# Kloudy-Sky/openintel

Hardware: AMD Instinct MI355X
Metric: queries/sec + p50 latency, 10M-post/768-d hybrid BM25+cosine+RRF top-100 (higher is better)
Workload: dtype f32

## Files before the change

### openintel_amd/csrc/cosine_screen_i8.hip

```cpp
#include <algorithm>
#include <cmath>
#include <cstdlib>
#include <type_traits>

#include "oi_device.h"
#include "oi_internal.h"
#include "oi_screen_stage.h"
#include "oi_lds_dma.h"

typedef int i8s_i32x4 __attribute__((ext_vector_type(4)));
typedef int i8s_i32x16 __attribute__((ext_vector_type(16)));
typedef float i8s_f32x2 __attribute__((ext_vector_type(2)));
template <int N>
struct i8s_ivec {
    typedef int type __attribute__((ext_vector_type(N)));
};

#define I8S_TILE_ROWS 32
#define I8S_SLOT_BYTES (I8S_TILE_ROWS * 128)
#define I8S_META_BYTES 256
#define I8S_PAD_ROWS 64

size_t oi_screen_i8_meta_offset(uint64_t n, uint32_t dim) { return ((size_t)n * dim + 255) & ~(size_t)255; }
size_t oi_screen_i8_bytes(uint64_t n, uint32_t dim) {
    return oi_screen_i8_meta_offset(n, dim) + 8 * ((size_t)n + I8S_PAD_ROWS) + 256;
}

__global__ __launch_bounds__(256) void i8s_make_kernel(const float *__restrict__ rows, uint64_t n, uint32_t dim,
                                                       const uint32_t *__restrict__ long_bitmap, uint32_t *__restrict__ out_i8,
                                                       float *__restrict__ meta, uint32_t *__restrict__ emax_bits) {
    const uint32_t lane = threadIdx.x & 63;
    const uint64_t wave = ((uint64_t)blockIdx.x * blockDim.x + threadIdx.x) >> 6;
    const uint64_t n_waves = ((uint64_t)gridDim.x * blockDim.x) >> 6;
    const uint32_t nv = dim >> 2;
    float best = 0.f;
    for (uint64_t r = wave; r < n; r += n_waves) {
        const float4 *x = reinterpret_cast<const float4 *>(rows + r * dim);
        float4 v[3];
        float amax = 0.f;
#pragma unroll
        for (int u = 0; u < 3; ++u) {
            const uint32_t j = lane + 64u * u;
            v[u] = j < nv ? x[j] : make_float4(0.f, 0.f, 0.f, 0.f);
            amax = fmaxf(amax, fmaxf(fmaxf(fabsf(v[u].x), fabsf(v[u].y)), fmaxf(fabsf(v[u].z), fabsf(v[u].w))));
        }
#pragma unroll
        for (int o = 32; o > 0; o >>= 1) amax = fmaxf(amax, __shfl_xor(amax, o, OI_WAVE));
        const float s = amax / 127.f;
        double e2 = 0.0;
#pragma unroll
        for (int u = 0; u < 3; ++u) {
            const uint32_t j = lane + 64u * u;
            const float xs[4] = {v[u].x, v[u].y, v[u].z, v[u].w};
            uint32_t packed = 0;
#pragma unroll
            for (int c = 0; c < 4; ++c) {
                float t = s > 0.f ? rintf(xs[c] / s) : 0.f;
                t = fminf(127.f, fmaxf(-127.f, t));
                const int iv = (int)t;
                const double e = (double)s * (double)iv - (double)xs[c];
                e2 += j < nv ? e * e : 0.0;
                packed |= ((uint32_t)iv & 0xFFu) << (8 * c);
            }
            if (j < nv) out_i8[r * nv + j] = packed;
        }
        e2 = oi_wave_sum(e2);
        const float er = (float)sqrt(e2) * 1.00000095367431640625f;
        if (lane == 0) {
            meta[2 * r] = s;
            meta[2 * r + 1] = er;
        }
        const bool is_long = long_bitmap && ((long_bitmap[r >> 5] >> (r & 31)) & 1u);
        if (!is_long) best = fmaxf(best, er);
    }
    if (lane == 0) atomicMax(emax_bits, __float_as_uint(best));
}

int oi_launch_make_screen_i8(oi_ctx *ctx, const float *rows, uint64_t n, uint32_t dim, const uint32_t *long_bitmap, uint8_t *out) {
    OI_REQUIRE(oi_cosine_screen_supported(dim), "int8 screening copy: dim %u not instantiated (384, 768)", dim);
    const size_t mo = oi_screen_i8_meta_offset(n, dim);
    OI_HIP_CHECK(hipMemsetAsync(out + mo, 0, 8 * ((size_t)n + I8S_PAD_ROWS) + 256, ctx->stream));
    if (n == 0) return OI_OK;
    uint64_t blocks = (n + 3) / 4;
    const uint64_t cap = (uint64_t)ctx->num_cus * 8;
    if (blocks > cap) blocks = cap;
    float *meta = reinterpret_cast<float *>(out + mo);
    hipLaunchKernelGGL(i8s_make_kernel, dim3((uint32_t)blocks), dim3(256), 0, ctx->stream, rows, n, dim, long_bitmap,
                       reinterpret_cast<uint32_t *>(out), meta, reinterpret_cast<uint32_t *>(meta + 2 * (n + I8S_PAD_ROWS)));
    OI_HIP_CHECK(hipGetLastError());
    return OI_OK;
}

#define I8S_NORM_LIMIT 1.0e15f
#define I8S_QNORM_MIN 1.0e-12f
__device__ __forceinline__ void i8s_stage_query_row(const float *__restrict__ q, uint32_t row, uint32_t n_queries, uint32_t n_padded, uint32_t dim,
                                                    const uint32_t *__restrict__ max_norm_bits, const uint32_t *__restrict__ emax_bits,
                                                    int8_t *__restrict__ qi8, float *__restrict__ qf, uint32_t *gate) {
    const uint32_t lane = threadIdx.x & 63;
    const bool real = row < n_queries;
    float amax = 0.f;
    bool fin = true;
    for (uint32_t k = lane; k < dim; k += 64) {
        const float f = real ? q[(uint64_t)row * dim + k] : 0.f;
        fin = fin && (f - f == 0.f);
        amax = fmaxf(amax, fabsf(f));
    }
#pragma unroll
    for (int o = 32; o > 0; o >>= 1) amax = fmaxf(amax, __shfl_xor(amax, o, OI_WAVE));
    fin = __builtin_amdgcn_ballot_w64(!fin) == 0ull;
    const float a = fin ? amax / 127.f : 0.f;
    double qn2 = 0.0, en2 = 0.0;
    for (uint32_t k = lane; k < dim; k += 64) {
        const float f = real ? q[(uint64_t)row * dim + k] : 0.f;
        float h = 0.f, l = 0.f;
        if (a > 0.f) {
            const float t = f / a;
            h = fminf(127.f, fmaxf(-127.f, rintf(t)));
            l = fminf(127.f, fmaxf(-127.f, rintf((t - h) * 128.f)));
        }
        const double qh = (double)a * ((double)h + (double)l * 0.0078125);
        qn2 += qh * qh;
        en2 += (qh - (double)f) * (qh - (double)f);
        qi8[(uint64_t)row * dim + k] = (int8_t)(int)h;
        qi8[((uint64_t)n_padded + row) * dim + k] = (int8_t)(int)l;
    }
    qn2 = oi_wave_sum(qn2);
    en2 = oi_wave_sum(en2);
    if (lane == 0) {
        const float up = 1.00000095367431640625f;
        const float qn = (float)sqrt(qn2) * up, en = (float)sqrt(en2) * up;
        const float X = __uint_as_float(max_norm_bits[0]), em = __uint_as_float(*emax_bits);
        const bool ok = fin && amax > 0.f && qn < I8S_NORM_LIMIT && qn >= I8S_QNORM_MIN && X < I8S_NORM_LIMIT && em < I8S_NORM_LIMIT;
        const float rnd = 3.814697265625e-06f + (float)dim * 2.384185791015625e-07f;
        const float cq = 1.001f * (X * en + rnd * (X + em) * (qn + en)) + 1.0e-27f;
        const float m2 = 2.002f * (em * qn + cq);
        qf[row] = ok ? a : 0.f;
        qf[n_padded + row] = ok ? qn : 0.f;
        qf[2 * n_padded + row] = ok ? cq : 0.f;
        qf[3 * n_padded + row] = ok || !real ? m2 : __builtin_inff();
        if (real && !ok) *gate = 1u;
    }
}
__global__ __launch_bounds__(256) void i8s_stage_kernel(const float *__restrict__ q, uint32_t n_queries, uint32_t n_padded, uint32_t dim,
                                                        const uint32_t *__restrict__ max_norm_bits, const uint32_t *__restrict__ emax_bits,
                                                        int8_t *__restrict__ qi8, float *__restrict__ qf, uint32_t *gate) {
    const uint32_t wave = (blockIdx.x * blockDim.x + threadIdx.x) >> 6, n_waves = (gridDim.x * blockDim.x) >> 6;
    for (uint32_t row = wave; row < n_padded; row += n_waves) {
        i8s_stage_query_row(q, row, n_queries, n_padded, dim, max_norm_bits, emax_bits, qi8, qf, gate);
    }
}

__global__ __launch_bounds__(256) void i8s_stage_both_kernel(const float *__restrict__ q, uint32_t n_queries, uint32_t n_padded, uint32_t dim,
                                                             const uint32_t *__restrict__ max_norm_bits, const uint32_t *__restrict__ emax_bits,
                                                             int8_t *__restrict__ qi8, float *__restrict__ qf, uint16_t *__restrict__ q_bf16,
                                                             float *__restrict__ eps2, uint32_t *gate) {
    const uint32_t wave = (blockIdx.x * blockDim.x + threadIdx.x) >> 6, n_waves = (gridDim.x * blockDim.x) >> 6;
    for (uint32_t row = wave; row < n_padded; row += n_waves) {
        i8s_stage_query_row(q, row, n_queries, n_padded, dim, max_norm_bits, emax_bits, qi8, qf, gate);
        pf_stage_query_row(q, row, n_queries, dim, max_norm_bits, q_bf16, eps2, gate);
    }
}

int oi_launch_screen_stage_i8(oi_ctx *ctx, const float *d_queries, uint32_t n_queries, uint32_t dim, const uint32_t *max_norm_bits,
                              const uint8_t *i8_copy, uint64_t n_rows, int8_t *qi8, float *qf, uint32_t *gate, uint16_t *q_bf16,
                              float *eps2) {
    const uint32_t n_padded = (n_queries + 31u) & ~31u;
    if (n_padded == 0) return OI_OK;
    const uint32_t *emax = reinterpret_cast<const uint32_t *>(i8_copy + oi_screen_i8_meta_offset(n_rows, dim)) + 2 * (n_rows + I8S_PAD_ROWS);
    if (q_bf16)
        hipLaunchKernelGGL(i8s_stage_both_kernel, dim3((n_padded + 3) / 4), dim3(256), 0, ctx->stream, d_queries, n_queries, n_padded, dim,
                           max_norm_bits, emax, qi8, qf, q_bf16, eps2, gate);
    else
        hipLaunchKernelGGL(i8s_stage_kernel, dim3((n_padded + 3) / 4), dim3(256), 0, ctx->stream, d_queries, n_queries, n_padded, dim,
                           max_norm_bits, emax, qi8, qf, gate);
    OI_HIP_CHECK(hipGetLastError());
    return OI_OK;
}

__device__ __forceinline__ void i8s_issue_piece(const oi_u32x4 &srd, uint32_t voff, uint32_t soff, uint32_t lds_dst) {
#ifdef I8S_NO_DMA
    (void)srd; (void)voff; (void)soff; (void)lds_dst;
#else
    oi_dma_piece(srd, voff, soff, lds_dst);
#endif
}
__device__ __forceinline__ void i8s_issue_meta(const oi_u32x4 &srd, uint32_t voff, uint32_t lds_dst) {
#ifdef I8S_NO_DMA
    (void)srd; (void)voff; (void)lds_dst;
#else
    uint32_t keep;
    const uint32_t d = __builtin_amdgcn_readfirstlane(lds_dst);
    asm volatile(
        "s_mov_b32 %0, m0\n\t"
        "s_mov_b32 m0, %3\n\t"
        "s_nop 0\n\t"
        "buffer_load_dword %1, %2, 0 offen " OI_DMA_NT "lds\n\t"
        "s_mov_b32 m0, %0"
        : "=&s"(keep)
        : "v"(voff), "s"(srd), "s"(d)
        : "memory");
#endif
}

template <int D, int NQT, int NBUF, bool FILT>
__global__ __launch_bounds__(256, 1) void cosine_i8_screen(
    const uint8_t *__restrict__ rows, const float *__restrict__ meta, uint64_t row_begin, uint64_t row_end,
    const int8_t *__restrict__ qhi, const int8_t *__restrict__ qlo,
    const float *__restrict__ qf, uint32_t qf_stride, uint32_t n_queries, uint32_t doc_id_base, uint64_t *pools, uint32_t *seg_cnt,
    uint32_t seg_cnt_stride, const uint32_t *tau_keys, uint64_t pool_stride, uint32_t carry_cap, uint32_t seg_cap, uint32_t *overflow,
    const uint4 *__restrict__ filt, const uint2 *__restrict__ attrs) {
    constexpr int NKC = D / 128;
    constexpr int P = NBUF - 1;
    constexpr int KSTEPS = D / 32;
    constexpr uint32_t RING = NBUF * I8S_SLOT_BYTES;
    static_assert(D % 128 == 0 && P >= 2 && P <= 2 * NKC, "unsupported ring depth for this D");
    constexpr uint32_t QLO_LDS = NQT * KSTEPS * 64 * 16;
    static_assert(NQT * KSTEPS * 4 <= 200, "the hi query block must fit the register file");
    static_assert(4 * RING + 4 * 2 * I8S_META_BYTES + 256 + OI_STAGE_LDS + QLO_LDS <= 160 * 1024, "LDS");

    extern __shared__ __attribute__((aligned(1024))) unsigned char smem[];
    unsigned char *ring = smem;
    unsigned char *meta_lds = smem + 4 * RING;
    uint32_t *seg_fill = reinterpret_cast<uint32_t *>(smem + 4 * RING + 8 * I8S_META_BYTES);
    unsigned char *stage_base = smem + 4 * RING + 8 * I8S_META_BYTES + 256;
    unsigned char *qlo_lds = stage_base + OI_STAGE_LDS;

    OI_CLAIM_WHOLE_SIMD();
    const uint32_t tid = threadIdx.x, lane = tid & 63;
    const uint32_t w = __builtin_amdgcn_readfirstlane(tid >> 6);
    const uint32_t li = lane & 31, lh = lane >> 5;
    uint64_t *stage_keys = reinterpret_cast<uint64_t *>(stage_base) + w * OI_STAGE;
    uint32_t *stage_q = reinterpret_cast<uint32_t *>(stage_base + 4 * OI_STAGE * 8) + w * OI_STAGE;
    uint32_t st_head = 0, st_n = 0;

    i8s_i32x4 qh[NQT][KSTEPS];
#pragma unroll
    for (int t = 0; t < NQT; ++t)
#pragma unroll
        for (int s = 0; s < KSTEPS; ++s)
            qh[t][s] = *reinterpret_cast<const i8s_i32x4 *>(qhi + (uint64_t)(32 * t + li) * D + 32 * s + 16 * lh);
    for (uint32_t c = tid; c < (uint32_t)(NQT * KSTEPS * 64); c += 256) {
        const uint32_t t = c / (KSTEPS * 64), s = (c / 64) % KSTEPS, l = c % 64;
        *reinterpret_cast<i8s_i32x4 *>(qlo_lds + c * 16) =
            *reinterpret_cast<const i8s_i32x4 *>(qlo + (uint64_t)(32 * t + (l & 31)) * D + 32 * s + 16 * (l >> 5));
    }
    float qa[NQT], qn[NQT], cq[NQT], tc[NQT];
#pragma unroll
    for (int t = 0; t < NQT; ++t) {
        const uint32_t q = 32u * t + li;
        const bool real = q < n_queries;
        const uint32_t k = real ? tau_keys[q] : 0xFFFFFFFFu;
        const float tau = k <= 0x007FFFFFu ? -__builtin_inff() : oi_key_f32(k);
        qa[t] = real ? qf[q] * 0.0078125f : 0.f;
        qn[t] = real ? qf[qf_stride + q] : 0.f;
        cq[t] = real ? qf[2 * qf_stride + q] : 0.f;
        const float m2 = real ? qf[3 * qf_stride + q] : 0.f;
        const float T = m2 < __builtin_inff() ? (tau + m2) - (fabsf(tau) + m2) * 9.5367431640625e-07f : -__builtin_inff();
        tc[t] = T - cq[t];
    }
    if (tid < 32 * NQT) seg_fill[tid] = 0;
#ifdef I8S_NO_DMA
    for (uint32_t i = tid; i < (4 * RING + 8 * I8S_META_BYTES) / 4; i += 256) reinterpret_cast<uint32_t *>(smem)[i] = 0u;
#endif
    __syncthreads();

    const uint64_t n_rows = row_end - row_begin;
    const uint64_t n_tiles = (n_rows + I8S_TILE_ROWS - 1) / I8S_TILE_ROWS;
    const uint64_t first = (uint64_t)blockIdx.x * 4 + w, stride = (uint64_t)gridDim.x * 4;
    const uint64_t my_nt = first < n_tiles ? (n_tiles - first + stride - 1) / stride : 0;
    uint64_t *my_seg = pools + carry_cap + (uint64_t)blockIdx.x * seg_cap;

    if (my_nt) {
        uint32_t voff[4];
#pragma unroll
        for (int m = 0; m < 4; ++m) {
            const uint32_t prow = 8 * m + (lane >> 3);
            voff[m] = prow * (uint32_t)D + (((lane & 7) ^ ((prow >> 1) & 7)) << 4);
        }
        const uint32_t ring_w = oi_lds_addr(ring) + w * RING;
        const unsigned char *ring_rd = ring + w * RING;
        const uint32_t meta_w = oi_lds_addr(meta_lds) + w * 2 * I8S_META_BYTES;
        const unsigned char *meta_rd = meta_lds + w * 2 * I8S_META_BYTES;
        uint32_t frag_off[4];
#pragma unroll
        for (int g = 0; g < 4; ++g) frag_off[g] = li * 128 + (((2 * g + lh) ^ ((li >> 1) & 7)) << 4);

        auto tile_row0 = [&](uint64_t ti) { return row_begin + (first + ti * stride) * (uint64_t)I8S_TILE_ROWS; };
        auto tile_srd = [&](uint64_t ti) {
            const uint64_t r0 = tile_row0(ti < my_nt ? ti : 0);
            return oi_make_srd(rows + r0 * D, ti < my_nt ? (row_end - r0) * (uint64_t)D : 0ull);
        };
        auto issue_meta = [&](uint64_t ti) {
            const uint64_t r0 = tile_row0(ti);
            i8s_issue_meta(oi_make_srd(meta + 2 * r0, (row_end - r0) * 8ull), lane * 4u, meta_w + (uint32_t)(ti & 1) * I8S_META_BYTES);
        };
        oi_u32x4 s0 = tile_srd(0), s1 = tile_srd(1), s2 = tile_srd(2);
        __builtin_amdgcn_s_waitcnt(0x0F70);
        oi_static_for<0, P>([&](auto j_) {
            constexpr int j = decltype(j_)::value;
            constexpr int tj = j / NKC, kj = j % NKC;
#pragma unroll
            for (int m = 0; m < 4; ++m)
                i8s_issue_piece(tj == 0 ? s0 : (tj == 1 ? s1 : s2), voff[m], kj * 128, ring_w + j * I8S_SLOT_BYTES + m * 1024);
        });
        issue_meta(0);
        uint32_t rd_off = 0, wr_off = (NBUF - 1) * I8S_SLOT_BYTES;
        auto lo_frag = [&](int t, int s) {
            return *reinterpret_cast<const i8s_i32x4 *>(qlo_lds + ((t * KSTEPS + s) * 64 + lane) * 16);
        };
        i8s_i32x4 b_cur[NQT];
#ifndef I8S_NO_MFMA
#pragma unroll
        for (int t = 0; t < NQT; ++t) b_cur[t] = lo_frag(t, 0);
#endif

        oi_wait_vm<4 * (P - 1)>();
        i8s_i32x4 a_cur = *reinterpret_cast<const i8s_i32x4 *>(ring_rd + frag_off[0]);

        constexpr int NS = 16 * NQT;
        constexpr int RPK = KSTEPS >= 20 ? 1 : 2;
        constexpr int NSL = 16 / RPK, T0 = 4;
        static_assert(T0 + NSL <= KSTEPS, "the tile test does not fit the span");
        static_assert(4 * NKC + 4 >= 4 * (P - 1) - 1, "the ring's wait in k-step 3 must retire the previous tile's metadata");
        typename i8s_ivec<NS>::type S;
#pragma unroll
        for (int i = 0; i < NS; ++i) S[i] = 0;
        i8s_i32x16 ah[NQT], al[NQT];
        i8s_f32x2 md_cur[RPK];
#pragma unroll
        for (int u = 0; u < RPK; ++u) md_cur[u] = i8s_f32x2{0.f, 0.f};
        const uint32_t lh32 = 32u * lh;
        auto meta_row = [&](const unsigned char *mt, int r) {
            return *reinterpret_cast<const i8s_f32x2 *>(mt + lh32 + ((r & 3) + 8 * (r >> 2)) * 8);
        };
        float cap_sc = 0.f, cap_er = 0.f;
        auto test_row = [&](int t, int r, const i8s_f32x2 md) -> uint32_t {
            const float sc = oi_mul_unpacked((float)S[16 * t + r], oi_mul_unpacked(md[0], qa[t]));
            const bool pass = sc >= oi_fma_unpacked(-md[1], qn[t], tc[t]);
            cap_sc = pass ? sc : cap_sc;
            cap_er = pass ? md[1] : cap_er;
            return pass ? 1u << (16 * t + r) : 0u;
        };

        for (uint64_t ti = 0;; ++ti) {
            const bool live = ti < my_nt;
            const unsigned char *mt = meta_rd + (uint32_t)((ti + 1) & 1) * I8S_META_BYTES;
            uint32_t m = 0;
            if (live) {
#pragma unroll
                for (int t = 0; t < NQT; ++t)
#pragma unroll
                    for (int r = 0; r < 16; ++r) { ah[t][r] = 0; al[t][r] = 0; }

                oi_static_for<0, NKC * 4>([&](auto gi_) {
                    constexpr int gi = decltype(gi_)::value;
                    constexpr int kc = gi / 4, g = gi % 4;
                    constexpr int sn = kc + P;
                    constexpr int tn = sn / NKC, kn = sn % NKC;
                    i8s_i32x4 a_nxt;
                    if constexpr (g < 3) {
                        a_nxt = *reinterpret_cast<const i8s_i32x4 *>(ring_rd + rd_off + frag_off[g + 1]);
                    } else {
                        oi_wait_vm<4 * (P - 1) - 1>();
                        const uint32_t nx_off = rd_off + I8S_SLOT_BYTES == RING ? 0u : rd_off + I8S_SLOT_BYTES;
                        a_nxt = *reinterpret_cast<const i8s_i32x4 *>(ring_rd + nx_off + frag_off[0]);
                    }
                    i8s_f32x2 md_nxt[RPK];
                    if constexpr (gi >= T0 - 1 && gi < T0 - 1 + NSL) {
#pragma unroll
                        for (int u = 0; u < RPK; ++u) md_nxt[u] = meta_row(mt, RPK * (gi - (T0 - 1)) + u);
                    }
#ifndef I8S_NO_MFMA
                    i8s_i32x4 b_nxt[NQT];
#pragma unroll
                    for (int t = 0; t < NQT; ++t) b_nxt[t] = lo_frag(t, (gi + 1) % KSTEPS);
#endif
                    __builtin_amdgcn_sched_barrier(0);
#pragma unroll
                    for (int t = 0; t < NQT; ++t) {
#ifndef I8S_NO_MFMA
                        ah[t] = __builtin_amdgcn_mfma_i32_32x32x32_i8(a_cur, qh[t][gi], ah[t], 0, 0, 0);
                        al[t] = __builtin_amdgcn_mfma_i32_32x32x32_i8(a_cur, b_cur[t], al[t], 0, 0, 0);
#else
                        asm volatile("" : : "v"(a_cur));
#endif
                        if constexpr (gi >= T0 && gi < T0 + NSL) if (t == 0) {
#pragma unroll
                            for (int u = 0; u < RPK; ++u)
#pragma unroll
                                for (int tt = 0; tt < NQT; ++tt) m |= test_row(tt, RPK * (gi - T0) + u, md_cur[u]);
                            asm volatile("" : "+v"(m), "+v"(cap_sc), "+v"(cap_er));
                        }
                        __builtin_amdgcn_sched_barrier(0);
                    }
#ifndef I8S_NO_MFMA
#pragma unroll
                    for (int t = 0; t < NQT; ++t) b_cur[t] = b_nxt[t];
#endif
                    if constexpr (gi >= T0 - 1 && gi < T0 - 1 + NSL) {
#pragma unroll
                        for (int u = 0; u < RPK; ++u) md_cur[u] = md_nxt[u];
                    }
                    i8s_issue_piece(tn == 0 ? s0 : (tn == 1 ? s1 : s2), voff[g], kn * 128, ring_w + wr_off + g * 1024);
                    if constexpr (g == 3) {
                        wr_off = rd_off;
                        rd_off = rd_off + I8S_SLOT_BYTES == RING ? 0u : rd_off + I8S_SLOT_BYTES;
                    }
                    a_cur = a_nxt;
                });
            } else {
                oi_wait_vm<0>();
#pragma unroll
                for (int r = 0; r < 16; ++r) {
                    const i8s_f32x2 md = meta_row(mt, r);
#pragma unroll
                    for (int t = 0; t < NQT; ++t) m |= test_row(t, r, md);
                }
            }

            const uint64_t row0 = tile_row0(ti ? ti - 1 : 0);
            if (ti == 0) m = 0u;
            const uint32_t m_tested = m;
            if (row_end - row0 < (uint64_t)I8S_TILE_ROWS) {
                const uint32_t left = (uint32_t)(row_end - row0);
#pragma unroll
                for (int r = 0; r < 16; ++r)
                    if ((uint32_t)((r & 3) + 8 * (r >> 2)) + 4u * lh >= left) m &= ~(0x00010001u << r);
            }
#if defined(I8S_NO_DMA) || defined(I8S_NO_MFMA) || defined(I8S_NO_APPEND)
            if (seg_cap != 0xFFFFFFFFu) m = 0u;
#endif
            if (__builtin_amdgcn_ballot_w64(m != 0u) != 0ull) {
                if constexpr (FILT) m = oi_filter_tile<NQT>(m, filt, attrs, row0, lh, li);
                static_assert(64u <= OI_STAGE - OI_STAGE_FLUSH, "a tile of one pair per lane must fit the staging ring");
                if (__builtin_amdgcn_ballot_w64((m_tested & (m_tested - 1u)) != 0u) == 0ull) {
                    const uint64_t has = __builtin_amdgcn_ballot_w64(m != 0u);
                    if (m != 0u) {
                        const uint32_t bit = (uint32_t)__builtin_ctz(m), r = bit & 15u;
                        const bool t1 = NQT > 1 && bit >= 16u;
                        const uint32_t rit = (r & 3) + 8 * (r >> 2) + 4 * lh;
                        const float low = cap_sc - fmaf(cap_er, t1 ? qn[NQT - 1] : qn[0], t1 ? cq[NQT - 1] : cq[0]);
                        const uint32_t below = __builtin_amdgcn_mbcnt_hi((uint32_t)(has >> 32), __builtin_amdgcn_mbcnt_lo((uint32_t)has, 0u));
                        const uint32_t idx = (st_head + st_n + below) & (OI_STAGE - 1);
                        stage_keys[idx] = oi_rank_key(low, doc_id_base + ((uint32_t)row0 + rit));
                        stage_q[idx] = (t1 ? 32u : 0u) + li;
                    }
                    st_n += (uint32_t)__builtin_popcountll(has);
                    while (st_n >= OI_STAGE_FLUSH) {
                        OI_STAGE_FLUSH_TO_POOL(OI_STAGE_FLUSH);
                    }
                } else {
                    const uint32_t cnt = (uint32_t)__builtin_popcount(m);
                    const uint32_t incl = oi_wave_incl_scan(cnt);
                    const uint32_t total = (uint32_t)__builtin_amdgcn_readlane((int)incl, 63);
                    const uint32_t any = oi_wave_or(m);
                    auto lower_key = [&](int t, uint32_t r) -> uint64_t {
                        const uint32_t rit = (r & 3) + 8 * (r >> 2) + 4 * lh;
                        const i8s_f32x2 md = *reinterpret_cast<const i8s_f32x2 *>(mt + rit * 8);
                        const float sc = (float)S[16 * t + r] * (md[0] * qa[t]);
                        return oi_rank_key(sc - fmaf(md[1], qn[t], cq[t]), doc_id_base + ((uint32_t)row0 + rit));
                    };
                    if (total <= OI_STAGE - OI_STAGE_FLUSH) {
                        uint32_t idx = st_head + st_n + incl - cnt;
#pragma unroll
                        for (int t = 0; t < NQT; ++t)
                            for (uint32_t wd = (any >> (16 * t)) & 0xFFFFu; wd; wd &= wd - 1) {
                                const uint32_t r = (uint32_t)__builtin_ctz(wd);
                                if (m & (1u << (16 * t + r))) {
                                    stage_keys[idx & (OI_STAGE - 1)] = lower_key(t, r);
                                    stage_q[idx & (OI_STAGE - 1)] = 32u * t + li;
                                    ++idx;
                                }
                            }
                        st_n += total;
                        while (st_n >= OI_STAGE_FLUSH) {
                            OI_STAGE_FLUSH_TO_POOL(OI_STAGE_FLUSH);
                        }
                    } else {
                        uint32_t pos[NQT];
#pragma unroll
                        for (int t = 0; t < NQT; ++t)
                            pos[t] = atomicAdd(&seg_fill[32u * t + li], (uint32_t)__builtin_popcount((m >> (16 * t)) & 0xFFFFu));
#pragma unroll
                        for (int t = 0; t < NQT; ++t) {
                            uint64_t *dst = my_seg + (uint64_t)(32u * t + li) * pool_stride;
                            for (uint32_t wd = (any >> (16 * t)) & 0xFFFFu; wd; wd &= wd - 1) {
                                const uint32_t r = (uint32_t)__builtin_ctz(wd);
                                if (m & (1u << (16 * t + r))) {
                                    if (pos[t] < seg_cap) dst[pos[t]] = lower_key(t, r);
                                    else *overflow = 1u;
                                    ++pos[t];
                                }
                            }
                        }
                    }
                }
            }
            if (!live) break;
#pragma unroll
            for (int t = 0; t < NQT; ++t)
#pragma unroll
                for (int r = 0; r < 16; ++r) S[16 * t + r] = ah[t][r] * 128 + al[t][r];
            if (ti + 1 < my_nt) issue_meta(ti + 1);
            s0 = s1;
            s1 = s2;
            s2 = tile_srd(ti + 3);
        }
        if (st_n) {
            OI_STAGE_FLUSH_TO_POOL(st_n);
        }
        oi_wait_vm<0>();
    }
    __syncthreads();
    if (tid < 32 * NQT && tid < n_queries) {
        const uint32_t c = seg_fill[tid];
        seg_cnt[(uint64_t)tid * seg_cnt_stride + blockIdx.x] = c < seg_cap ? c : seg_cap;
    }
}

template <int D, int NQT, int NBUF, bool FILT>
static int launch_i8_screen_k(oi_ctx *ctx, const uint8_t *rows, const float *meta, uint64_t row_begin, uint64_t row_end, const int8_t *qhi,
                              const int8_t *qlo, const float *qf, uint32_t qf_stride, uint32_t nq, uint32_t doc_id_base, const PoolView &p) {
    constexpr size_t smem = 4 * NBUF * I8S_SLOT_BYTES + 8 * I8S_META_BYTES + 256 + OI_STAGE_LDS + NQT * (D / 32) * 64 * 16;
    OI_CHECK(oi_dyn_lds(ctx, reinterpret_cast<const void *>(cosine_i8_screen<D, NQT, NBUF, FILT>), (size_t)(smem)));
    hipLaunchKernelGGL((cosine_i8_screen<D, NQT, NBUF, FILT>), dim3(p.n_segs), dim3(256), smem, ctx->stream, rows, meta, row_begin, row_end,
                       qhi, qlo, qf, qf_stride, nq, doc_id_base, p.keys, p.seg_cnt, p.seg_cnt_stride, p.tau_keys, p.stride, p.carry_cap,
                       p.seg_cap, p.overflow, p.filt, p.attrs);
    OI_HIP_CHECK(hipGetLastError());
    return OI_OK;
}
template <int D, int NQT, int NBUF>
static int launch_i8_screen(oi_ctx *ctx, const uint8_t *rows, const float *meta, uint64_t row_begin, uint64_t row_end, const int8_t *qhi,
                            const int8_t *qlo, const float *qf, uint32_t qf_stride, uint32_t nq, uint32_t doc_id_base, const PoolView &p) {
    return p.filt ? launch_i8_screen_k<D, NQT, NBUF, true>(ctx, rows, meta, row_begin, row_end, qhi, qlo, qf, qf_stride, nq, doc_id_base, p)
                  : launch_i8_screen_k<D, NQT, NBUF, false>(ctx, rows, meta, row_begin, row_end, qhi, qlo, qf, qf_stride, nq, doc_id_base, p);
}

int oi_launch_cosine_screen_i8_chunk(oi_ctx *ctx, const uint8_t *i8_copy, uint64_t n_rows_total, uint64_t row_begin, uint64_t row_end,
                                     uint32_t dim, const int8_t *qi8, const float *qf, uint32_t n_queries, uint32_t doc_id_base,
                                     PoolView &pool) {
    OI_REQUIRE(oi_cosine_screen_supported(dim), "cosine screen (int8): dim %u not instantiated (384, 768)", dim);
    OI_REQUIRE(row_end <= n_rows_total, "cosine screen (int8): rows past the copy");
    oi_cosine_screen_geometry(ctx, row_end > row_begin ? row_end - row_begin : 0, &pool.n_segs, &pool.seg_cap);
    OI_REQUIRE(pool.n_segs <= pool.seg_cnt_stride && pool.carry_cap + (uint64_t)pool.n_segs * pool.seg_cap <= pool.stride,
               "cosine screen (int8): chunk does not fit the candidate pool");
    if (row_end <= row_begin || n_queries == 0) return OI_OK;
    const float *meta = reinterpret_cast<const float *>(i8_copy + oi_screen_i8_meta_offset(n_rows_total, dim));
    const uint32_t np = (n_queries + 31u) & ~31u;
    ProfScope ps(ctx, "cosine");
    for (uint32_t q0 = 0; q0 < n_queries; q0 += 64) {
        const uint32_t nq_here = std::min(64u, n_queries - q0);
        const PoolView p = pool.for_queries(q0);
        const int8_t *qhi = qi8 + (uint64_t)q0 * dim, *qlo = qi8 + ((uint64_t)np + q0) * dim;
        const float *qfp = qf + q0;
        const bool two = nq_here > 32;
        if (dim == 768) {
            if (two) OI_CHECK((launch_i8_screen<768, 2, 6>(ctx, i8_copy, meta, row_begin, row_end, qhi, qlo, qfp, np, nq_here, doc_id_base, p)));
            else OI_CHECK((launch_i8_screen<768, 1, 6>(ctx, i8_copy, meta, row_begin, row_end, qhi, qlo, qfp, np, nq_here, doc_id_base, p)));
        } else {
            if (two) OI_CHECK((launch_i8_screen<384, 2, 6>(ctx, i8_copy, meta, row_begin, row_end, qhi, qlo, qfp, np, nq_here, doc_id_base, p)));
            else OI_CHECK((launch_i8_screen<384, 1, 6>(ctx, i8_copy, meta, row_begin, row_end, qhi, qlo, qfp, np, nq_here, doc_id_base, p)));
        }
    }
    return OI_OK;
}

__device__ __forceinline__ float i8s_bf16_lo(uint32_t w) { return __uint_as_float(w << 16); }
__device__ __forceinline__ float i8s_bf16_hi(uint32_t w) { return __uint_as_float(w & 0xFFFF0000u); }
__global__ __launch_bounds__(256) void pf_rescreen_kernel(const uint16_t *__restrict__ copy, uint64_t n_rows, uint32_t dim,
                                                          uint32_t doc_id_base, const uint16_t *__restrict__ qb, uint64_t *pools,
                                                          const uint32_t *__restrict__ cnt, uint64_t stride, uint32_t cap) {
    const uint32_t q = blockIdx.y, lane = threadIdx.x & 63;
    const uint32_t wave = (blockIdx.x * blockDim.x + threadIdx.x) >> 6, n_waves = (gridDim.x * blockDim.x) >> 6;
    uint32_t c = cnt[q];
    c = c < cap ? c : cap;
    uint64_t *keys = pools + (uint64_t)q * stride;
    const uint32_t nvec = dim >> 3;
    const uint4 *qv = reinterpret_cast<const uint4 *>(qb + (uint64_t)q * dim);
    for (uint32_t i0 = wave * 4u; i0 < c; i0 += n_waves * 4u) {
        uint32_t doc[4];
        const uint4 *x[4];
        float a[4];
#pragma unroll
        for (int u = 0; u < 4; ++u) {
            const uint32_t i = i0 + u < c ? i0 + u : c - 1u;
            doc[u] = oi_rank_key_doc(keys[i]);
            const uint64_t r = (uint64_t)(doc[u] - doc_id_base);
            x[u] = reinterpret_cast<const uint4 *>(copy + (r < n_rows ? r : 0) * dim);
            a[u] = 0.f;
        }
        for (uint32_t v = lane; v < nvec; v += 64) {
            const uint4 yv = qv[v];
            uint4 xv[4];
#pragma unroll
            for (int u = 0; u < 4; ++u) xv[u] = oi_load_stream(x[u] + v);
#pragma unroll
            for (int u = 0; u < 4; ++u) {
                const uint32_t xw[4] = {xv[u].x, xv[u].y, xv[u].z, xv[u].w}, yw[4] = {yv.x, yv.y, yv.z, yv.w};
#pragma unroll
                for (int e = 0; e < 4; ++e) {
                    a[u] = oi_fma_unpacked(i8s_bf16_lo(xw[e]), i8s_bf16_lo(yw[e]), a[u]);
                    a[u] = oi_fma_unpacked(i8s_bf16_hi(xw[e]), i8s_bf16_hi(yw[e]), a[u]);
                }
            }
        }
        float s[4];
#pragma unroll
        for (int u = 0; u < 4; ++u) s[u] = oi_wave_sum(a[u]);
#pragma unroll
        for (int u = 0; u < 4; ++u) {
            const uint64_t r = (uint64_t)(doc[u] - doc_id_base);
            const float sc = r < n_rows ? s[u] : 0.f;
            if (lane == 0 && i0 + u < c) keys[i0 + u] = oi_rank_key(sc, doc[u]);
        }
    }
}

int oi_launch_rescreen_bf16(oi_ctx *ctx, const uint16_t *copy_rows, uint64_t n_rows, uint32_t dim, uint32_t doc_id_base,
                            const uint16_t *q_bf16, uint32_t n_queries, const PoolView &pool) {
    if (n_queries == 0) return OI_OK;
    ProfScope ps(ctx, "rescreen");
    hipLaunchKernelGGL(pf_rescreen_kernel, dim3(32, n_queries), dim3(256), 0, ctx->stream, copy_rows, n_rows, dim, doc_id_base, q_bf16,
                       pool.keys, pool.carry_cnt, pool.stride, pool.carry_cap);
    OI_HIP_CHECK(hipGetLastError());
    return OI_OK;
}
```

### openintel_amd/csrc/select.hip

```cpp
#include "oi_device.h"
#include "oi_internal.h"

#define SEL_THREADS 1024
#define SEL_MAX 1024

__device__ void bitonic_sort_desc(uint64_t *a, uint32_t P) {
    const uint32_t tid = threadIdx.x;
    for (uint32_t size = 2; size <= P; size <<= 1) {
        for (uint32_t stride = size >> 1; stride > 0; stride >>= 1) {
            for (uint32_t t = tid; t < (P >> 1); t += SEL_THREADS) {
                uint32_t lo = 2 * t - (t & (stride - 1));
                uint32_t hi = lo + stride;
                bool desc = ((lo & size) == 0);
                uint64_t x = a[lo], y = a[hi];
                if ((x < y) == desc) { a[lo] = y; a[hi] = x; }
            }
            __syncthreads();
        }
    }
}

#define SEL_LDS_KEYS 8192

struct SelSource {
    const uint64_t *pool;
    const uint32_t *segc;
    const uint64_t *lds_keys;
    uint32_t n, c0, carry_cap, seg_cap, n_segs;
};

template <class F>
__device__ __forceinline__ void sel_for_each(const SelSource &S, F &&f) {
    const uint32_t tid = threadIdx.x;
    if (S.lds_keys) {
        for (uint32_t i = tid; i < S.n; i += SEL_THREADS) f(S.lds_keys[i]);
        return;
    }
    for (uint32_t i = tid; i < S.c0; i += SEL_THREADS) f(S.pool[i]);
    const uint32_t lane = tid & 63, wv = tid >> 6;
    for (uint32_t sg = wv; sg < S.n_segs; sg += SEL_THREADS / 64) {
        uint32_t c = S.segc[sg];
        if (c > S.seg_cap) c = S.seg_cap;
        const uint64_t *base = S.pool + S.carry_cap + (uint64_t)sg * S.seg_cap;
        for (uint32_t i = lane; i < c; i += 64) f(base[i]);
    }
}

__global__ __launch_bounds__(SEL_THREADS) void select_topk_kernel(
    uint64_t *pools, uint32_t *carry_cnt, uint32_t *seg_cnt, uint32_t *tau_keys, uint64_t pool_stride,
    uint32_t carry_cap, uint32_t seg_cap, uint32_t n_segs, uint32_t seg_cnt_stride, uint32_t *overflow,
    uint32_t k, int compact, float *out_scores, uint32_t *out_docs, uint32_t *out_counts, uint32_t out_stride) {
    __shared__ uint32_t hist[256];
    __shared__ uint64_t sel[2 * SEL_MAX];
    __shared__ uint64_t lds_keys[SEL_LDS_KEYS];
    __shared__ uint32_t s_cnt, s_kk, s_bin_cnt, s_total;
    __shared__ uint64_t s_prefix;

    const uint32_t q = blockIdx.x, tid = threadIdx.x;
    uint64_t *pool = pools + (uint64_t)q * pool_stride;
    uint32_t *segc = seg_cnt + (uint64_t)q * seg_cnt_stride;
    SelSource S;
    S.pool = pool; S.segc = segc; S.lds_keys = nullptr;
    S.carry_cap = carry_cap; S.seg_cap = seg_cap; S.n_segs = n_segs;
    S.c0 = carry_cnt[q] < carry_cap ? carry_cnt[q] : carry_cap;
    if (tid == 0) { s_cnt = 0; s_total = 0; }
    __syncthreads();
    {
        uint32_t local = 0;
        for (uint32_t sg = tid; sg < n_segs; sg += SEL_THREADS) {
            uint32_t c = segc[sg];
            if (c > seg_cap) { *overflow = 1u; c = seg_cap; }
            local += c;
        }
        local = oi_wave_sum(local);
        if ((tid & 63) == 0 && local) atomicAdd(&s_total, local);
    }
    __syncthreads();
    const uint32_t n = S.c0 + s_total;
    S.n = n;
    if (n <= SEL_LDS_KEYS) {
        sel_for_each(S, [&](uint64_t key) { lds_keys[atomicAdd(&s_cnt, 1u)] = key; });
        __syncthreads();
        S.lds_keys = lds_keys;
        if (tid == 0) s_cnt = 0;
        __syncthreads();
    }

    uint32_t m;
    if (n <= k) {
        sel_for_each(S, [&](uint64_t key) { sel[atomicAdd(&s_cnt, 1u)] = key; });
        m = n;
        __syncthreads();
    } else {
        if (tid == 0) { s_prefix = 0; s_kk = k; }
        int shift = 56;
        for (;; shift -= 8) {
            if (tid < 256) hist[tid] = 0;
            __syncthreads();
            const uint64_t prefix = s_prefix;
            if (shift == 56)
                sel_for_each(S, [&](uint64_t key) { atomicAdd(&hist[(uint32_t)(key >> 56)], 1u); });
            else
                sel_for_each(S, [&](uint64_t key) {
                    if ((key >> (shift + 8)) == prefix) atomicAdd(&hist[(uint32_t)(key >> shift) & 255u], 1u);
                });
            __syncthreads();
            if (tid < 64) {
                const uint32_t kk = s_kk;
                uint32_t mine = 0;
                for (int i = 0; i < 4; ++i) mine += hist[255 - (tid * 4 + i)];
                uint32_t incl = mine;
#pragma unroll
                for (int o = 1; o < 64; o <<= 1) {
                    uint32_t v = __shfl_up(incl, o, OI_WAVE);
                    if ((int)tid >= o) incl += v;
                }
                const unsigned long long ball = __ballot(incl >= kk);
                const uint32_t owner = ball ? (uint32_t)__builtin_ctzll(ball) : 63u;
                if (tid == owner) {
                    uint32_t cum = incl - mine;
                    int d = 255 - (int)(tid * 4);
                    for (int i = 0; i < 3; ++i, --d) {
                        const uint32_t c = hist[d];
                        if (cum + c >= kk) break;
                        cum += c;
                    }
                    s_prefix = (prefix << 8) | (uint64_t)d;
                    s_kk = kk - cum;
                    s_bin_cnt = hist[d];
                }
            }
            __syncthreads();
            if (s_bin_cnt == 1 || shift == 0) break;
        }
        const uint64_t prefix = s_prefix;
        sel_for_each(S, [&](uint64_t key) {
            if ((key >> shift) >= prefix) {
                const uint32_t pos = atomicAdd(&s_cnt, 1u);
                if (pos < SEL_MAX) sel[pos] = key;
            }
        });
        __syncthreads();
        m = s_cnt < k ? s_cnt : k;
    }
    __shared__ unsigned long long s_min;
    if (out_scores) {
        uint32_t P = 2;
        while (P < m) P <<= 1;
        for (uint32_t i = m + tid; i < P; i += SEL_THREADS) sel[i] = 0;
        __syncthreads();
        bitonic_sort_desc(sel, P);
        for (uint32_t i = tid; i < m; i += SEL_THREADS) {
            const uint64_t key = sel[i];
            out_scores[(uint64_t)q * out_stride + i] = oi_rank_key_score(key);
            out_docs[(uint64_t)q * out_stride + i] = oi_rank_key_doc(key);
        }
        if (tid == 0) { out_counts[q] = m; s_min = m ? sel[m - 1] : 0; }
    } else {
        if (tid == 0) s_min = ~0ull;
        __syncthreads();
        unsigned long long lo = ~0ull;
        for (uint32_t i = tid; i < m; i += SEL_THREADS) lo = sel[i] < lo ? sel[i] : lo;
#pragma unroll
        for (int o = 32; o > 0; o >>= 1) {
            const unsigned long long v = __shfl_xor(lo, o, OI_WAVE);
            lo = v < lo ? v : lo;
        }
        if ((tid & 63) == 0 && lo != ~0ull) atomicMin(&s_min, lo);
    }
    __syncthreads();
    if (compact) {
        for (uint32_t i = tid; i < m; i += SEL_THREADS) pool[i] = sel[i];
        for (uint32_t sg = tid; sg < n_segs; sg += SEL_THREADS) segc[sg] = 0;
        if (tid == 0) {
            carry_cnt[q] = m;
            if (m == k && tau_keys) {
                const uint32_t t = (uint32_t)(s_min >> 32);
                if (t > tau_keys[q]) tau_keys[q] = t;
            }
        }
    }
}

#define SEL_MAX_SEGS 4096
#define SEL_KPT_MAX 32
#ifdef OI_ABLATION
__device__ int sel_dbg_on;
__device__ unsigned long long sel_dbg_t[16];
#define SEL_STAMP(i) do { if (sel_dbg_on && blockIdx.x == 0 && threadIdx.x == 0) sel_dbg_t[i] = __builtin_readcyclecounter(); } while (0)
#else
#define SEL_STAMP(i) do { } while (0)
#endif
#define SEL_CAND 4096

struct SelRowMargin {
    const float *meta;
    uint32_t base;
    float qn, cq;
};
__device__ __forceinline__ float sel_row_e(const SelRowMargin *rm, uint64_t kv) {
    return rm->meta[2 * (uint64_t)(oi_rank_key_doc(kv) - rm->base) + 1];
}
__device__ __forceinline__ bool sel_row_test(const SelRowMargin *rm, uint64_t kv, float e, float edge, float eps2) {
    const float u = oi_rank_key_score(kv) + 2.002f * (e * rm->qn + rm->cq);
    return u >= edge - 9.5367431640625e-07f * (fabsf(edge) + eps2);
}
__device__ __forceinline__ bool sel_row_keep(const SelRowMargin *rm, uint64_t kv, float edge, float eps2) {
    if (!rm) return true;
    return sel_row_test(rm, kv, sel_row_e(rm, kv), edge, eps2);
}

__device__ __forceinline__ void sel_spec_words(bool have, uint32_t rth_key, float eps2, uint32_t tau, uint32_t *spec_tau, uint32_t *spec_max) {
    if (!have) { *spec_tau = tau; return; }
    const float s = oi_key_f32(rth_key) - eps2;
    const uint32_t T = s == s ? oi_f32_key(s) : 0u;
    const uint32_t st = T > tau ? T : tau;
    *spec_tau = st;
    if (st > tau && st > *spec_max) *spec_max = st;
}

struct SelShared {
    uint32_t hist[256];
    uint32_t hist2k[2048];
    uint32_t seg_off[SEL_MAX_SEGS + 1];
    uint32_t wave_tot[SEL_THREADS / 64];
    uint32_t cnt, kk, bin_cnt, n_samples;
    uint64_t prefix;
    unsigned long long min_key;
};

struct SelFlat {
    const uint64_t *pool;
    const uint32_t *seg_off;
    uint32_t n, c0, carry_cap, seg_cap, n_segs, steps;
};
struct SelCursor {
    uint32_t sg, lo, hi;
};
__device__ __forceinline__ SelCursor sel_seek(const SelFlat &K, uint32_t i) {
    const uint32_t e = i < K.c0 ? 0u : i - K.c0;
    uint32_t lo = 0, hi = K.n_segs;
    for (uint32_t s = 0; s < K.steps; ++s) {
        const uint32_t mid = (lo + hi) >> 1;
        const bool up = K.seg_off[mid] <= e;
        lo = up ? mid : lo;
        hi = up ? hi : mid;
    }
    SelCursor c;
    c.sg = lo; c.lo = K.seg_off[lo]; c.hi = K.seg_off[lo + 1];
    return c;
}
__device__ __forceinline__ uint64_t sel_at(const SelFlat &K, SelCursor &c, uint32_t i) {
    if (i < K.c0) return i;
    const uint32_t e = i - K.c0;
    while (e >= c.hi) {
        ++c.sg;
        c.lo = c.hi;
        c.hi = K.seg_off[c.sg + 1];
    }
    return (uint64_t)K.carry_cap + (uint64_t)c.sg * K.seg_cap + (e - c.lo);
}

__device__ __forceinline__ void sel_hist_add(uint32_t *hist, bool active, uint32_t digit) {
    const uint32_t lane = threadIdx.x & 63;
#pragma unroll
    for (int r = 0; r < 2; ++r) {
        const unsigned long long m = __ballot(active);
        if (!m) return;
        const uint32_t leader = (uint32_t)__builtin_ctzll(m);
        const uint32_t d0 = (uint32_t)__shfl((int)digit, (int)leader, OI_WAVE);
        const unsigned long long same = __ballot(active && digit == d0);
        if (lane == leader) atomicAdd(&hist[d0], (uint32_t)__popcll(same));
        active = active && digit != d0;
    }
    if (active) atomicAdd(&hist[digit], 1u);
}

__device__ __forceinline__ void sel_append(uint64_t *dst, uint32_t *count, uint32_t cap, bool take, uint64_t key) {
    const unsigned long long m = __ballot(take);
    if (!m) return;
    const uint32_t lane = threadIdx.x & 63, leader = (uint32_t)__builtin_ctzll(m);
    uint32_t base = 0;
    if (lane == leader) base = atomicAdd(count, (uint32_t)__popcll(m));
    base = (uint32_t)__shfl((int)base, (int)leader, OI_WAVE);
    const uint32_t pos = base + (uint32_t)__popcll(m & ((1ull << lane) - 1ull));
    if (take && pos < cap) dst[pos] = key;
}

__device__ __forceinline__ void sel_hist_add_w(uint32_t *hist, bool active, uint32_t digit, uint32_t weight) {
    const uint32_t lane = threadIdx.x & 63;
#pragma unroll
    for (int r = 0; r < 2; ++r) {
        const unsigned long long m = __ballot(active);
        if (!m) return;
        const uint32_t leader = (uint32_t)__builtin_ctzll(m);
        const uint32_t d0 = (uint32_t)__builtin_amdgcn_readlane((int)digit, (int)leader);
        const bool same = active && digit == d0;
        const uint32_t sum = (uint32_t)__builtin_amdgcn_readlane((int)oi_wave_incl_scan(same ? weight : 0u), 63);
        if (lane == leader) atomicAdd(&hist[d0], sum);
        active = active && !same;
    }
    if (active) atomicAdd(&hist[digit], weight);
}

template <class FE>
__device__ __forceinline__ void sel_threshold(FE &&for_each, uint32_t kk_in, SelShared &sh, int &shift_out, uint64_t &prefix_out) {
    const uint32_t tid = threadIdx.x;
    if (tid == 0) { sh.prefix = 0; sh.kk = kk_in; }
    int shift = 56;
    for (;; shift -= 8) {
        if (tid < 256) sh.hist[tid] = 0;
        __syncthreads();
        const uint64_t prefix = sh.prefix;
        const bool top = shift == 56;
        for_each([&](bool valid, uint64_t kv) {
            sel_hist_add(sh.hist, valid && (top || (kv >> ((shift + 8) & 63)) == prefix), (uint32_t)(kv >> shift) & 255u);
        });
        __syncthreads();
        if (tid < 64) {
            const uint32_t kk = sh.kk;
            uint32_t mine = 0;
            for (int i = 0; i < 4; ++i) mine += sh.hist[255 - (tid * 4 + i)];
// ... 671 lines not shown
```

Baseline: 35630.

## Software-pipeline rescreen gathers and use in-register bitonic sort stages

```diff
diff --git a/openintel_amd/csrc/cosine_screen_i8.hip b/openintel_amd/csrc/cosine_screen_i8.hip
--- a/openintel_amd/csrc/cosine_screen_i8.hip
+++ b/openintel_amd/csrc/cosine_screen_i8.hip
@@ -7,6 +7,7 @@
 #include "oi_internal.h"
 #include "oi_screen_stage.h"
 #include "oi_lds_dma.h"
+#include "oi_gather_trips.h"
 
 typedef int i8s_i32x4 __attribute__((ext_vector_type(4)));
 typedef int i8s_i32x16 __attribute__((ext_vector_type(16)));
@@ -567,6 +568,34 @@
 
 __device__ __forceinline__ float i8s_bf16_lo(uint32_t w) { return __uint_as_float(w << 16); }
 __device__ __forceinline__ float i8s_bf16_hi(uint32_t w) { return __uint_as_float(w & 0xFFFF0000u); }
+__device__ __forceinline__ float i8s_bf16_fma8(const uint4 &xv, const uint4 &yv, float a) {
+    const uint32_t xw[4] = {xv.x, xv.y, xv.z, xv.w}, yw[4] = {yv.x, yv.y, yv.z, yv.w};
+#pragma unroll
+    for (int e = 0; e < 4; ++e) {
+        a = oi_fma_unpacked(i8s_bf16_lo(xw[e]), i8s_bf16_lo(yw[e]), a);
+        a = oi_fma_unpacked(i8s_bf16_hi(xw[e]), i8s_bf16_hi(yw[e]), a);
+    }
+    return a;
+}
+template <uint32_t DIM>
+__device__ __forceinline__ void pf_rescreen_trips(const uint16_t *__restrict__ copy, uint64_t n_rows, uint32_t doc_id_base,
+                                                  const uint4 *__restrict__ qv, uint64_t *keys, uint32_t c, uint32_t wave,
+                                                  uint32_t n_waves, uint32_t lane) {
+    oi_gather_trips<DIM / 8, uint4>(
+        qv, c, wave, n_waves, lane,
+        [&](uint32_t i) { return reinterpret_cast<const uint32_t *>(keys)[2 * (uint64_t)i]; },
+        [&](uint32_t, uint32_t raw) { return ~raw; },
+        [&](uint32_t doc) {
+            const uint64_t r = (uint64_t)(doc - doc_id_base);
+            return reinterpret_cast<const uint4 *>(copy + (r < n_rows ? r : 0) * DIM);
+        },
+        [&](const uint4 &x, const uint4 &y, float a) { return i8s_bf16_fma8(x, y, a); },
+        [&](uint32_t i, uint32_t doc, float a) {
+            const uint64_t r = (uint64_t)(doc - doc_id_base);
+            const float s = oi_wave_sum(a);
+            if (lane == 0) keys[i] = oi_rank_key(r < n_rows ? s : 0.f, doc);
+        });
+}
 __global__ __launch_bounds__(256) void pf_rescreen_kernel(const uint16_t *__restrict__ copy, uint64_t n_rows, uint32_t dim,
                                                           uint32_t doc_id_base, const uint16_t *__restrict__ qb, uint64_t *pools,
                                                           const uint32_t *__restrict__ cnt, uint64_t stride, uint32_t cap) {
@@ -577,6 +606,8 @@
     uint64_t *keys = pools + (uint64_t)q * stride;
     const uint32_t nvec = dim >> 3;
     const uint4 *qv = reinterpret_cast<const uint4 *>(qb + (uint64_t)q * dim);
+    if (dim == 768) return pf_rescreen_trips<768>(copy, n_rows, doc_id_base, qv, keys, c, wave, n_waves, lane);
+    if (dim == 384) return pf_rescreen_trips<384>(copy, n_rows, doc_id_base, qv, keys, c, wave, n_waves, lane);
     for (uint32_t i0 = wave * 4u; i0 < c; i0 += n_waves * 4u) {
         uint32_t doc[4];
         const uint4 *x[4];
@@ -595,14 +626,7 @@
 #pragma unroll
             for (int u = 0; u < 4; ++u) xv[u] = oi_load_stream(x[u] + v);
 #pragma unroll
-            for (int u = 0; u < 4; ++u) {
-                const uint32_t xw[4] = {xv[u].x, xv[u].y, xv[u].z, xv[u].w}, yw[4] = {yv.x, yv.y, yv.z, yv.w};
-#pragma unroll
-                for (int e = 0; e < 4; ++e) {
-                    a[u] = oi_fma_unpacked(i8s_bf16_lo(xw[e]), i8s_bf16_lo(yw[e]), a[u]);
-                    a[u] = oi_fma_unpacked(i8s_bf16_hi(xw[e]), i8s_bf16_hi(yw[e]), a[u]);
-                }
-            }
+            for (int u = 0; u < 4; ++u) a[u] = i8s_bf16_fma8(xv[u], yv, a[u]);
         }
         float s[4];
 #pragma unroll
diff --git a/openintel_amd/csrc/oi_gather_trips.h b/openintel_amd/csrc/oi_gather_trips.h
--- /dev/null
+++ b/openintel_amd/csrc/oi_gather_trips.h
@@ -0,0 +1,65 @@
+#pragma once
+#include "oi_device.h"
+
+template <uint32_t NV, class Vec, class RawAt, class DocOf, class RowOf, class Fma, class Put>
+__device__ __forceinline__ void oi_gather_trips(const Vec *__restrict__ qv, uint32_t c, uint32_t wave, uint32_t n_waves, uint32_t lane,
+                                                RawAt &&raw_at, DocOf &&doc_of, RowOf &&row_of, Fma &&fma, Put &&put) {
+    constexpr uint32_t NP = (NV + 63) / 64;
+    struct Trip {
+        uint32_t raw[4], doc[4];
+        Vec x[4][NP];
+    };
+    const uint32_t step = n_waves * 4u;
+    uint32_t i0 = wave * 4u;
+    if (i0 >= c) return;
+    Vec yv[NP];
+#pragma unroll
+    for (uint32_t p = 0; p < NP; ++p) yv[p] = qv[lane + 64 * p < NV ? lane + 64 * p : NV - 1];
+    auto slot = [&](uint32_t i) { return i < c ? i : c - 1u; };
+    auto ask = [&](Trip &t, uint32_t i) {
+#pragma unroll
+        for (int u = 0; u < 4; ++u) t.raw[u] = raw_at(slot(i + u));
+    };
+    auto fetch = [&](Trip &t, uint32_t i) {
+#pragma unroll
+        for (int u = 0; u < 4; ++u) t.doc[u] = doc_of(slot(i + u), t.raw[u]);
+#pragma unroll
+        for (uint32_t p = 0; p < NP; ++p)
+#pragma unroll
+            for (int u = 0; u < 4; ++u) t.x[u][p] = oi_load_stream(row_of(t.doc[u]) + (lane + 64 * p < NV ? lane + 64 * p : NV - 1));
+    };
+    auto finish = [&](const Trip &t, uint32_t i) {
+#pragma unroll
+        for (int u = 0; u < 4; ++u) {
+            float a = 0.f;
+#pragma unroll
+            for (uint32_t p = 0; p < NP; ++p)
+                if (64 * p + 64 <= NV || lane + 64 * p < NV) a = fma(t.x[u][p], yv[p], a);
+            if (i + u < c) put(i + u, t.doc[u], a);
+        }
+    };
+    Trip A, B;
+    uint32_t s0 = (uint32_t)__builtin_amdgcn_readfirstlane((int)i0);
+    const uint32_t cs = (uint32_t)__builtin_amdgcn_readfirstlane((int)c);
+    ask(A, i0);
+    ask(B, i0 + step);
+    __builtin_amdgcn_sched_barrier(0);
+    fetch(A, i0);
+#pragma unroll
+    for (int u = 0; u < 4; ++u) asm volatile("" ::"v"(B.raw[u]));
+    while (s0 + step < cs) {
+        ask(A, i0 + 2 * step);
+        __builtin_amdgcn_sched_barrier(0);
+        fetch(B, i0 + step);
+        __builtin_amdgcn_sched_barrier(0);
+        finish(A, i0);
+        ask(B, i0 + 3 * step);
+        __builtin_amdgcn_sched_barrier(0);
+        fetch(A, i0 + 2 * step);
+        __builtin_amdgcn_sched_barrier(0);
+        finish(B, i0 + step);
+        i0 += 2 * step;
+        s0 += 2 * step;
+    }
+    if (s0 < cs) finish(A, i0);
+}
diff --git a/openintel_amd/csrc/select.hip b/openintel_amd/csrc/select.hip
--- a/openintel_amd/csrc/select.hip
+++ b/openintel_amd/csrc/select.hip
@@ -4,20 +4,68 @@
 #define SEL_THREADS 1024
 #define SEL_MAX 1024
 
+template <int STRIDE>
+__device__ __forceinline__ uint32_t sort_lane_xor(uint32_t v) {
+    if constexpr (STRIDE == 1) return (uint32_t)__builtin_amdgcn_update_dpp(0, (int)v, 0xB1, 0xf, 0xf, false);
+    else if constexpr (STRIDE == 2) return (uint32_t)__builtin_amdgcn_update_dpp(0, (int)v, 0x4E, 0xf, 0xf, false);
+    else if constexpr (STRIDE < 32) return (uint32_t)__builtin_amdgcn_ds_swizzle((int)v, (STRIDE << 10) | 0x1f);
+    else return (uint32_t)__builtin_amdgcn_ds_bpermute((int)(((threadIdx.x & 63u) ^ 32u) << 2), (int)v);
+}
+template <int STRIDE>
+__device__ __forceinline__ void sort_lane_stages(uint64_t &key, bool down) {
+    const uint64_t p = ((uint64_t)sort_lane_xor<STRIDE>((uint32_t)(key >> 32)) << 32) | sort_lane_xor<STRIDE>((uint32_t)key);
+    const bool keep_max = ((threadIdx.x & STRIDE) == 0) == down;
+    key = (p > key) == keep_max ? p : key;
+    if constexpr (STRIDE > 1) sort_lane_stages<STRIDE / 2>(key, down);
+}
+template <int SIZE>
+__device__ __forceinline__ void sort_lane_merges(uint64_t &key, uint32_t idx, uint32_t P) {
+    if constexpr (SIZE > 2) sort_lane_merges<SIZE / 2>(key, idx, P);
+    if (SIZE <= P) sort_lane_stages<SIZE / 2>(key, (idx & SIZE) == 0);
+}
 __device__ void bitonic_sort_desc(uint64_t *a, uint32_t P) {
     const uint32_t tid = threadIdx.x;
-    for (uint32_t size = 2; size <= P; size <<= 1) {
-        for (uint32_t stride = size >> 1; stride > 0; stride >>= 1) {
+    const bool two = P > SEL_THREADS;
+    const bool live = (tid & ~63u) < P;
+    uint64_t e0 = tid < P ? a[tid] : 0, e1 = two ? a[tid + SEL_THREADS] : 0;
+    if (live) {
+        sort_lane_merges<64>(e0, tid, P);
+        if (two) sort_lane_merges<64>(e1, tid + SEL_THREADS, P);
+    }
+    for (uint32_t size = 128; size <= P; size <<= 1) {
+        uint32_t stride = size >> 1;
+        if (stride == SEL_THREADS) {
+            const uint64_t x = e0, y = e1;
+            e0 = x < y ? y : x;
+            e1 = x < y ? x : y;
+            stride >>= 1;
+        }
+        if (live) {
+            a[tid] = e0;
+            if (two) a[tid + SEL_THREADS] = e1;
+        }
+        __syncthreads();
+        for (; stride >= 64; stride >>= 1) {
             for (uint32_t t = tid; t < (P >> 1); t += SEL_THREADS) {
-                uint32_t lo = 2 * t - (t & (stride - 1));
-                uint32_t hi = lo + stride;
-                bool desc = ((lo & size) == 0);
-                uint64_t x = a[lo], y = a[hi];
+                const uint32_t lo = 2 * t - (t & (stride - 1)), hi = lo + stride;
+                const bool desc = (lo & size) == 0;
+                const uint64_t x = a[lo], y = a[hi];
                 if ((x < y) == desc) { a[lo] = y; a[hi] = x; }
             }
             __syncthreads();
         }
-    }
+        if (live) {
+            e0 = a[tid];
+            sort_lane_stages<32>(e0, (tid & size) == 0);
+            if (two) {
+                e1 = a[tid + SEL_THREADS];
+                sort_lane_stages<32>(e1, ((tid + SEL_THREADS) & size) == 0);
+            }
+        }
+    }
+    if (tid < P) a[tid] = e0;
+    if (two) a[tid + SEL_THREADS] = e1;
+    if (P > 64) __syncthreads();
 }
 
 #define SEL_LDS_KEYS 8192
```

New measurement: 36110 (median of 6 runs). 1.01x the previous value.
